# dubhater/vapoursynth-mvtools

Hardware: AMD Instinct MI355X
Metric: MDegrain3 cfg3 fps (Super+Analyse+Degrain end-to-end) (higher is better)
Workload: dtype u16; 1 GPU; 4K YUV420P16 Degrain3 blksize=16 overlap=8 pel=2; batches_in_flight=2

## Files before the change

include/mvtools_amd.h:

```cpp
#ifndef MVTOOLS_AMD_H
#define MVTOOLS_AMD_H

#include <stddef.h>
#include <stdint.h>

#ifdef __cplusplus
extern "C" {
#endif

#define MVX_UNSET (-2147483647 - 1)
#define MVX_ERRLEN 256

#define MVX_OK 0
#define MVX_E_ARG (-1)
#define MVX_E_DEVICE (-2)
#define MVX_E_NOMEM (-3)

const char *mvx_last_error(void);
int mvx_device_count(void);
const char *mvx_version(void);


typedef struct mvx_vector { int32_t x, y; int64_t sad; } mvx_vector;

// ... 570 lines not shown
    float motion[4];
    mvx_depan_stabilise_source prev, next;
} mvx_depan_stabilise_frame_plan;

typedef struct mvx_depan_stabilise mvx_depan_stabilise;

int mvx_depan_stabilise_create(const mvx_depan_stabilise_args *args, const mvx_depan_clip *clip, int num_frames, int data_frames,
                               int64_t fps_num, int64_t fps_den, const ptrdiff_t src_pitch[3], const ptrdiff_t dst_pitch[3],
                               mvx_depan_stabilise **out, char *err);
void mvx_depan_stabilise_destroy(mvx_depan_stabilise *h);
void mvx_depan_stabilise_get_info(const mvx_depan_stabilise *h, mvx_depan_stabilise_info *info);
void mvx_depan_stabilise_get_windows(const mvx_depan_stabilise *h, float *wint, float *winrz, float *winfz);
int mvx_depan_stabilise_window(const mvx_depan_stabilise *h, int n, int *data_first, int *data_last, int *clip_first, int *clip_last);
int mvx_depan_stabilise_plan(const mvx_depan_stabilise *h, int n, const float *motions, mvx_depan_stabilise_frame_plan *plan, char *err);

typedef struct mvx_depan_stabilise_job {
    mvx_depan_stabilise_frame_plan plan;
    const void *cur[3];
    const void *prev[3];
    const void *next[3];
    void *dst[3];
} mvx_depan_stabilise_job;

int mvx_depan_stabilise_frames(mvx_depan_stabilise *h, int nframes, const mvx_depan_stabilise_job *jobs, void *stream);

int mvx_scdetect(const mvx_analysis_data *vectors_data, int64_t thscd1, int32_t thscd2, int n, const void *const *blobs,
                 int32_t *scene_change, void *stream, char *err);

void mvx_scale_thscd(int64_t *thscd1, int32_t *thscd2, const mvx_analysis_data *ad);
int mvx_vectors_size(const mvx_analysis_data *ad);

int mvx_debug_option(const char *name, int value);
void mvx_debug_last_launch(int out[5]);
int mvx_analyse_dct_blocks(mvx_analyse *a, const void *plane, ptrdiff_t pitch, int n, const int32_t *xs, const int32_t *ys, void *out_bytes, void *stream);

void *mvx_dev_alloc(size_t bytes);
void *mvx_dev_alloc_uninit(size_t bytes);
void mvx_dev_free(void *p);
void mvx_dev_pool_limit(size_t bytes);
void mvx_dev_pool_trim(void);
int mvx_dev_mem_info(size_t *free_bytes, size_t *total_bytes);
void *mvx_stream_create(void);
void *mvx_stream_create_priority(int level);
void mvx_stream_destroy(void *stream);
int mvx_copy_to_device(void *dst, ptrdiff_t dst_pitch, const void *src_host, ptrdiff_t src_pitch, size_t row_bytes, size_t rows, void *stream);
int mvx_copy_to_host(void *dst_host, ptrdiff_t dst_pitch, const void *src, ptrdiff_t src_pitch, size_t row_bytes, size_t rows, void *stream);
int mvx_stream_sync(void *stream);
void *mvx_host_alloc_pinned(size_t bytes);
void mvx_host_free_pinned(void *p);
int mvx_upload_2d(void *dst, ptrdiff_t dst_pitch, const void *src_host, ptrdiff_t src_pitch, size_t row_bytes, size_t rows, void *stream);
int mvx_download_2d(void *dst_host, ptrdiff_t dst_pitch, const void *src, ptrdiff_t src_pitch, size_t row_bytes, size_t rows, void *stream);
int mvx_dev_memset(void *dst, int value, size_t bytes, void *stream);
int mvx_set_device(int ordinal);
int mvx_warmup(int staging_buffers);

#ifdef __cplusplus
}
#endif
#endif
```

vapoursynth-mvtools_amd/build.py:

```python
import os
import subprocess
import sys

HERE = os.path.dirname(os.path.abspath(__file__))
CSRC = os.path.join(HERE, "csrc")
OUT = os.path.join(HERE, "libmvtools_amd.so")
SOURCES = ["mvx_api.hip", "mvx_super.hip", "mvx_analyse.hip", "mvx_analyse_any.hip", "mvx_analyse_fdct.hip", "mvx_analyse_u8.hip", "mvx_analyse_u16.hip", "mvx_analyse_spec_u8.hip", "mvx_analyse_spec_u16.hip", "mvx_degrain.hip", "mvx_degrain_n.hip", "mvx_compensate_n.hip", "mvx_flow.hip", "mvx_mask.hip", "mvx_depan.hip", "mvx_depan_fft.hip", "mvx_depan_warp.hip", "mvx_scale_vect.hip"]
FLAGS = ["--offload-arch=gfx950", "-O3", "-std=c++17", "-ffp-contract=off", "-fPIC", "-fvisibility=hidden", "-Wall", "-Wno-inline-asm",
         "-Wno-unused-function", "-Wno-unused-variable"]
if os.environ.get("MVX_DEFS"):
    FLAGS += ["-D" + d for d in os.environ["MVX_DEFS"].split()]
if os.environ.get("MVX_PROFILE"):
    FLAGS.append("-DMVX_PROFILE")


def _hipcc():
    for c in (os.environ.get("HIPCC"), "/opt/rocm/bin/hipcc", "hipcc"):
        if c and (os.path.isabs(c) and os.path.exists(c) or not os.path.isabs(c)):
            return c
    return "hipcc"


VSDIR = os.path.join(HERE, "vsplugin")
VS_PLUGIN = os.path.join(HERE, "libmvtools_vs.so")
VS_HOST = os.path.join(HERE, "mvx_vs_host")


def build_vs(force=False, verbose=False):
    srcs = [os.path.join(VSDIR, f) for f in os.listdir(VSDIR)] + [os.path.join(HERE, "..", "include", "mvtools_amd.h")]
    if not force and all(os.path.exists(o) and all(os.path.getmtime(d) <= os.path.getmtime(o) for d in srcs) for o in (VS_PLUGIN, VS_HOST)):
        return VS_PLUGIN, VS_HOST
    cc = os.environ.get("CC", "gcc")
    cmds = [[cc, "-std=gnu11", "-O2", "-Wall", "-Wextra", "-fPIC", "-shared", "-fvisibility=hidden", os.path.join(VSDIR, "mvtools_vs.c"), "-o", VS_PLUGIN,
             "-L" + HERE, "-lmvtools_amd", "-Wl,-rpath,$ORIGIN", "-lpthread"],
            [cc, "-std=gnu11", "-O2", "-Wall", "-Wextra", os.path.join(VSDIR, "minihost.c"), "-o", VS_HOST, "-ldl"]]
    for cmd in cmds:
        if verbose:
            print(" ".join(cmd))
        subprocess.check_call(cmd)
    return VS_PLUGIN, VS_HOST
# ... 39 lines not shown
```

vapoursynth-mvtools_amd/csrc/mvx_analyse.hip:

```cpp
#include <stdarg.h>
#include <stdlib.h>

#include <algorithm>
#include "mvx_analyse_kernel.h"
#include "mvx_analyse_fast.h"
#include "mvx_analyse_spec.h"
#include "mvx_dct_host.h"
int mvx_analyse_launch_spec_u8(const AParams &P, const ASpecLaunch &S);
int mvx_analyse_launch_spec_u16(const AParams &P, const ASpecLaunch &S);


static thread_local char g_err[512];
void mvx_set_error(const char *fmt, ...) {
    va_list ap;
    va_start(ap, fmt);
    vsnprintf(g_err, sizeof(g_err), fmt, ap);
    va_end(ap);
}
extern "C" __attribute__((visibility("default"))) const char *mvx_last_error(void) { return g_err; }

struct MvxDebug {
    int general = 0;
    int cpw1 = 0;
    int spec = 1;
    int team = -1;
};
static MvxDebug g_dbg;
extern "C" __attribute__((visibility("default"))) int mvx_debug_option(const char *name, int value) {
    struct { const char *n; int *p; } tab[] = { { "general", &g_dbg.general }, { "cpw1", &g_dbg.cpw1 }, { "spec", &g_dbg.spec }, { "team", &g_dbg.team } };
    for (auto &t : tab) if (!strcmp(t.n, name)) { *t.p = value; return MVX_OK; }
    mvx_set_error("mvx_debug_option: unknown option %s", name);
    return MVX_E_ARG;
}

static std::atomic<int> g_lastLaunch[5];
extern "C" __attribute__((visibility("default"))) void mvx_debug_last_launch(int out[5]) {
    for (int i = 0; i < 5; i++) out[i] = g_lastLaunch[i].load();
}

static int A(int v, int d) { return v == MVX_UNSET ? d : v; }

static std::atomic<int> g_dctFloat{0};
extern "C" __attribute__((visibility("default"))) int mvx_enable_dct_float(int on) {
    g_dctFloat.store(on ? 1 : 0);
    return MVX_OK;
}
static bool mvx_is_fdct(const AParams &P) { return P.dctmode >= 1 && P.dctmode <= 4; }
static int mvx_dct_upload(AParams &P, float **dTab) {
    if (!mvx_is_fdct(P) || *dTab) return MVX_OK;
    const std::vector<float> t = mvx_dct_tables(P.blkX, P.blkY);
    HIP_CHECK(hipMalloc((void **)dTab, t.size() * sizeof(float)));
    HIP_CHECK(hipMemcpy(*dTab, t.data(), t.size() * sizeof(float), hipMemcpyHostToDevice));
    P.dctTab = *dTab;
    return MVX_OK;
}

void mvx_divided_data(const mvx_analysis_data *in, mvx_analysis_data *out) {
    *out = *in;
    out->nBlkX = in->nBlkX * 2; out->nBlkY = in->nBlkY * 2;
    out->nBlkSizeX = in->nBlkSizeX / 2; out->nBlkSizeY = in->nBlkSizeY / 2;
    out->nOverlapX = in->nOverlapX / 2; out->nOverlapY = in->nOverlapY / 2;
    out->nLvCount = in->nLvCount + 1;
}

__device__ __forceinline__ int mvx_median3(int a, int b, int c) {
    if (((b <= a) && (a <= c)) || ((c <= a) && (a <= b))) return a;
    if (((a <= b) && (b <= c)) || ((c <= b) && (b <= a))) return b;
    return c;
// ... 230 lines not shown
    (void)hipFree(dXY);
    return rc;
}

extern "C" __attribute__((visibility("default"))) int mvx_analyse_frames(mvx_analyse *a, int njobs, const mvx_analyse_job *jobs, void *stream) {
    if (njobs <= 0) return MVX_OK;
    hipStream_t st = (hipStream_t)stream;
    if (int rc0 = mvx_analyse_device_state(a)) return rc0;
    const AParams &P = a->P;
    mvx_analyse::JobSlot &S = a->slot[a->nextSlot.fetch_add(1) % mvx_analyse::kSlots];
    CallGuard::Scope scope(S.guard, st);
    if ((size_t)njobs > S.cap) {
        if (S.d) (void)hipFree(S.d);
        S.cap = (size_t)njobs * 2;
        HIP_CHECK(hipMalloc((void **)&S.d, S.cap * sizeof(AJob)));
    }
    std::vector<AJob> hj(njobs);
    for (int i = 0; i < njobs; i++) {
        for (int p = 0; p < 3; p++) { hj[i].src[p] = (const unsigned char *)jobs[i].src[p]; hj[i].ref[p] = (const unsigned char *)jobs[i].ref[p]; }
        hj[i].blob = (unsigned char *)jobs[i].blob;
        hj[i].fieldShift = jobs[i].field_shift;
        hj[i].valid = jobs[i].ref[0] != nullptr;
        if (((uintptr_t)jobs[i].blob) & 15) { mvx_set_error("mvx_analyse_frames: blob must be 16-byte aligned"); return MVX_E_ARG; }
    }
    if (!g_dbg.cpw1) std::stable_sort(hj.begin(), hj.end(), [](const AJob &x, const AJob &y) { return (uintptr_t)x.ref[0] > (uintptr_t)y.ref[0]; });
    HIP_CHECK(hipMemcpyAsync(S.d, hj.data(), sizeof(AJob) * njobs, hipMemcpyHostToDevice, st));
    int simds = 0;
    {
        int dev = 0, cus = 0;
        HIP_CHECK(hipGetDevice(&dev));
        HIP_CHECK(hipDeviceGetAttribute(&cus, hipDeviceAttributeMultiprocessorCount, dev));
        simds = 4 * cus;
    }
    auto finish = [&](int fast, int cpw, int syncEvery, int kind) {
        g_lastLaunch[0] = fast; g_lastLaunch[1] = cpw; g_lastLaunch[2] = syncEvery; g_lastLaunch[3] = njobs; g_lastLaunch[4] = kind;
        if (P.divide) hipLaunchKernelGGL(analyse_divide_kernel, dim3((P.lv[0].nBlkX * P.lv[0].nBlkY + 255) / 256, njobs), dim3(256), 0, st, a->dP, S.d);
        HIP_CHECK(hipGetLastError());
        return MVX_OK;
    };
    if (mvx_fast_eligible(P) && !g_dbg.general && !g_dbg.cpw1) {
        int srcB = P.blkX * P.blkY * P.bps + 2 * (P.blkX / 2) * (P.blkY / 2) * P.bps;
        const int fRow = (srcB + 15) & ~15;
        int fMaxBlkX = 0;
        for (int i = 0; i < P.nLevels; i++) if (P.lv[i].nBlkX > fMaxBlkX) fMaxBlkX = P.lv[i].nBlkX;
        const int fBins = 1024;
        int fNeed = fRow + fMaxBlkX * 16;
        if (fNeed < fRow + fBins * 4) fNeed = fRow + fBins * 4;
        const bool stripShape8 = P.bps == 1 && P.blkX == 8 && P.chroma && (P.ovX == 4 || P.ovX == 0) && P.shadow[1] != 0;
        const bool uvOrLumaOnly = P.chroma ? P.shadow[1] != 0 : true;
        const bool stripShape16 = P.bps == 1 && P.blkX == 16 && uvOrLumaOnly && (P.ovX == 8 || P.ovX == 0);
        const bool stripShape = (P.bps == 2 && (P.blkX == 16 || (MVX_STRIP32 && P.blkX == 32)) && uvOrLumaOnly && (P.ovX == P.blkX / 2 || (P.blkX == 16 && P.ovX == 0))) || stripShape8 || stripShape16;
        const int sStrip = (P.bps == 2 && P.blkX == 16) ? 2 * 24 * 128  : (P.bps == 2 && MVX_STRIP32 && P.blkX == 32) ? (P.blkX + P.blkX / 2) * 128 : (P.bps == 1 && P.blkX == 16) ? 24 * 64 : 0;
        const int sSrc = stripShape8 ? 16 + 768 : fRow < sStrip ? sStrip : fRow;
        int sNeed = 0, sTabMax = 0;
        for (int i = 0; i < P.nLevels; i++) {
            const bool smallest = i == P.nLevels - 1;
            const int st = smallest ? (P.nLevels == 1 ? P.searchType : P.searchTypeCoarse) : (i == 0 ? P.searchType : P.searchTypeCoarse);
            const int tabB = (st == SearchHex2 ? SPEC_SLOTS_HEX : SPEC_SLOTS_EXH) * SPEC_STRIDE;
            const int need = sSrc + ((P.lv[i].nBlkX * 8 + 15) & ~15) + tabB;
            if (need > sNeed) sNeed = need;
            if (tabB > sTabMax) sTabMax = tabB;
        }
        if (sNeed < sSrc + fBins * 4) sNeed = sSrc + fBins * 4;
        const int teamShared = (64 + fMaxBlkX * 8 + 255) & ~255;
        const int teamPerWave = ((sSrc + sTabMax < sSrc + fBins * 4 ? sSrc + fBins * 4 : sSrc + sTabMax) + 255) & ~255;
        auto teamThatFits = [&](int team) {
            if (team == 1 || team > 8) team = 0;
// ... 5 lines not shown
        const bool useSpecStrips = useSpec && g_dbg.spec != 3 && stripShape;
        int sTab = 0, sRow = fRow;
        if (useSpec) {
            sRow = sSrc;
            sTab = sSrc + ((fMaxBlkX * 8 + 15) & ~15);
            fNeed = sNeed;
        }
        const int perChain = (fNeed + 255) & ~255;
        auto have = [&](int k) {
            if (P.bps == 2 && P.blkX == 8) return k == 1 || k == 2 || k == 4;
            if (P.bps == 2 && P.blkX == 32) return k >= 1 && k <= 3;
            return k >= 1 && k <= 4;
        };
        int k = njobs > 3 * simds ? 4 : njobs > 2 * simds ? 3 : njobs > simds ? 2 : 1;
        if (useSpecStrips && k > 2) k = 2;
        while (k > 1 && (!have(k) || (long long)perChain * 4 * k > 160 * 1024)) k--;
        if ((long long)perChain * 4 * k <= 160 * 1024) {
            const int cpw = useSpecStrips ? 4 : 4 * k;
            int syncEvery = k >= 2 ? (P.bps == 2 ? 32 : 256) : 0;
            if (useSpecStrips) syncEvery = (stripShape8 || stripShape16) ? 0 : 128;
            const int flags = MVX_FAST_XCD_REMAP | ((P.shadow[1] != 0 && P.chroma) ? MVX_FAST_UV : 0) | (g_dbg.spec == 2 ? MVX_FAST_NOSPEC : 0) | (g_dbg.spec == 3 ? MVX_FAST_NOSTRIP : 0);
            const ALaunch L = { njobs, 0, useSpec ? sRow : fRow, useSpec ? sRow : fRow, fBins, fNeed, simds, cpw, k, syncEvery, k, flags, st, a->dP, S.d };
            int rc;
            const int specSide = ((P.blkX == 16 || stripShape8) && P.ovX == 0) ? 1 : 0;
            const int team = useSpec ? teamThatFits(g_dbg.team >= 0 ? g_dbg.team : mvx_team_default(njobs, simds, useSpecStrips, P.bps)) : 0;
            if (team) {
                ALaunch TL = L;
                TL.ldsRow = teamShared; TL.ldsNeed = teamPerWave; TL.ldsHist = sRow; TL.syncEvery = 0; TL.fast = 2; TL.cpw = 1;
                const ASpecLaunch SL = { TL, sRow, team, specSide };
                rc = P.bps == 1 ? mvx_analyse_launch_spec_u8(P, SL) : mvx_analyse_launch_spec_u16(P, SL);
                if (rc == MVX_OK) return finish(2, team, 0, 3);
                if (rc != 1) return rc;
            }
            if (useSpec) { const ASpecLaunch SL = { L, sTab, 0, specSide }; rc = P.bps == 1 ? mvx_analyse_launch_spec_u8(P, SL) : mvx_analyse_launch_spec_u16(P, SL); }
            else rc = P.bps == 1 ? mvx_analyse_launch_fast_u8(P, L) : mvx_analyse_launch_fast_u16(P, L);
            if (rc == MVX_OK) return finish(k, cpw, syncEvery, useSpec ? 2 : 0);
            if (rc != 1) return rc;
        }
    }
    const bool specialised = P.dctmode == 0 && P.xr == 2 && P.yr == 2 && P.blkX == P.blkY && (P.blkX == 16 || P.blkX == 8 || (P.blkX == 32 && P.bps == 2));
    int cpw = g_dbg.cpw1 ? 1 : 4, wpe = 1;
    if (specialised && !g_dbg.cpw1 && njobs > simds) {
        if (P.bps == 1 && (P.blkX == 8 || P.blkX == 16)) wpe = 2;
        if (P.bps == 1 && P.blkX == 8 && njobs > 2 * simds) wpe = 3;
        if (P.bps == 2 && (P.blkX == 16 || P.blkX == 8 || P.blkX == 32)) { wpe = 2; cpw = 8; }
    }
    int srcBytes = P.blkX * P.blkY * P.bps;
    if (P.chroma) srcBytes += 2 * (P.blkX / P.xr) * (P.blkY / P.yr) * P.bps;
    int ldsRow = (srcBytes + 15) & ~15;
    int maxBlkX = 0;
    for (int i = 0; i < P.nLevels; i++) if (P.lv[i].nBlkX > maxBlkX) maxBlkX = P.lv[i].nBlkX;
    const int histBins = 1024;
    const int ldsHist = ldsRow + maxBlkX * 16;
    int ldsBytes = ldsHist + histBins * 4;
    if (mvx_is_fdct(P)) ldsBytes += mvx_dct_lds_bytes(P.blkX, P.blkY);
    if (ldsBytes > 160 * 1024) { mvx_set_error("mvx_analyse_frames: frame too wide for the LDS row buffer"); return MVX_E_ARG; }
    const int ldsNeed = ldsBytes;
    if (ldsBytes < 33 * 1024) ldsBytes = 33 * 1024;
    while (cpw > 1 && (long long)((ldsNeed + 255) & ~255) * cpw > 160 * 1024) {
        cpw = cpw == 8 ? 4 : 1;
        if (wpe == 3) wpe = 2;
        if (P.bps == 2) wpe = 1;
    }
    const int syncEvery = wpe >= 2 ? 256 : 0;
    const ALaunch L = { njobs, ldsBytes, ldsRow, ldsHist, histBins, ldsNeed, simds, cpw, wpe, syncEvery, 0, 0, st, a->dP, S.d };
    bool off32 = true;
// ... 180 lines not shown
```

vapoursynth-mvtools_amd/csrc/mvx_analyse_spec.h:

```cpp
#pragma once
#include <type_traits>
#include "mvx_analyse_fast.h"

#define SPEC_TB 32
#define SPEC_STRIDE (SPEC_TB * 8 + 8)
#define SPEC_SLOTS_HEX 19
#define SPEC_SLOTS_EXH 29
#define MVX_FAST_NOSTRIP 8
#define MVX_FAST_NOSPEC 4

constexpr int SPEC_SW3 = 12;
#ifdef MVX_SPEC_PROF
#define SPROF_N 20
static __device__ unsigned long long g_specprof[SPROF_N];
#define SPROF(i) do { const long long t1_ = (long long)__builtin_amdgcn_s_memtime(); asm volatile("s_waitcnt lgkmcnt(0)" : : "s"(t1_) : "memory"); sprof[i] += t1_ - sprofT; sprofT = t1_; } while (0)
#else
#define SPROF(i) ((void)0)
#endif
#ifdef MVX_SPEC_PROF
#define SPEC_PROF_DUMP_() do { if (l == 0 && chain == 5 && S.role == 1) for (int i = 0; i < SPROF_N; i++) g_specprof[i] = (unsigned long long)S.sprof[i]; } while (0)
#else
#define SPEC_PROF_DUMP_() ((void)0)
#endif
#ifdef MVX_SPEC_STATS
static __device__ unsigned long long g_specstat[MVX_MAX_LEVELS][8];
#endif

template <int BPS, int BW, bool UV, int SWIN = 12, bool TEAM = false, bool SIDE = false> struct SpecSearcher : FastSearcher<BPS, BW, UV, 48> {
    typedef FastSearcher<BPS, BW, UV, 48> F;
    typedef FGeo<BPS, BW> G;
    using F::P; using F::J; using F::lds; using F::ldsRow; using F::ldsHist; using F::histBins;
    using F::nBlkX; using F::nBlkY; using F::pel; using F::logPel; using F::pw; using F::ph; using F::hpad; using F::vpad;
    using F::srcY; using F::srcU; using F::srcV; using F::refY; using F::refU; using F::refV; using F::srcUV; using F::refUV;
    using F::pitchY; using F::pitchC; using F::pstrideY; using F::pstrideC; using F::shadowY; using F::vectors;
    using F::chroma; using F::searchType; using F::nSearchParam; using F::penaltyNew; using F::penaltyZero; using F::pglobal; using F::badrange; using F::badcount; using F::fieldShift;
    using F::badSAD; using F::LSAD; using F::gmvx; using F::gmvy;
    using F::x0; using F::y0; using F::blkIdx; using F::nDxMin; using F::nDyMin; using F::nDxMax; using F::nDyMax;
    using F::predX; using F::predY; using F::pX; using F::pY; using F::nLambda; using F::bestX; using F::bestY; using F::bestSad;
    int ldsTab;
    int role, nw;
    lds_u8 *shRow;
    LDS_AS int *ctl;
    __device__ __forceinline__ int team_advance(int g, int c0, int lo, int hiE, bool fwd, int stepX, int hps) const {
        auto clampAt = [&](int v, int li) { const int xb = stepX * (c0 + li); return min(max(v, -((xb + hps) << logPel)), ((pw - xb - hpad - BW - hpad + hps) << logPel) - 1); };
        if (clampAt(g, lo) == g && clampAt(g, hiE - 1) == g) return g;
        for (int i = 0; i < hiE - lo; i++) g = clampAt(g, fwd ? lo + i : hiE - 1 - i);
        return g;
    }
    __device__ __forceinline__ void team_wait_ge(int need) const {
#ifdef MVX_TEAM_WATCHDOG
        unsigned spins = 0;
#endif
        while (uni(__hip_atomic_load(ctl, __ATOMIC_ACQUIRE, __HIP_MEMORY_SCOPE_WORKGROUP)) < need) {
            __builtin_amdgcn_s_sleep(2);
#ifdef MVX_TEAM_WATCHDOG
            if (++spins > (1u << 26)) __builtin_trap();
#endif
        }
    }
    __device__ __forceinline__ void team_acquire(int myG, int &px, int &py, int &ps) {
        team_wait_ge(myG);
// ... 178 lines not shown
            a0 = t ? b2 : b0; a1 = t ? b3 : b1; a2 = t ? b0 : b2; a3 = t ? b1 : b3;
        };
        rot(aL0, aL1, aL2, aL3, shA); rot(aC0, aC1, aC2, aC3, shB);
        T.aL[0] = aL0; T.aL[1] = aL1; T.aL[2] = aL2; T.aL[3] = aL3; T.aC[0] = aC0; T.aC[1] = aC1; T.aC[2] = aC2; T.aC[3] = aC3;
    }
    __device__ __forceinline__ static void pat_delta(bool hex, int idx, int &dx, int &dy) {
        dx = 0; dy = 0;
        if (hex) {
            if (idx < 6) { dx = tab8(HEX2X >> 8, idx & 7); dy = tab8(HEX2Y >> 8, idx & 7); }
            else if (idx < 14) { dx = tab8(PACK8(0, 0, -1, 1, -1, -1, 1, 1), idx - 6); dy = tab8(PACK8(-1, 1, 0, 0, -1, 1, -1, 1), idx - 6); }
        } else {
            if (idx < 8) { dx = tab8(PACK8(0, 0, -1, 1, -1, -1, 1, 1), idx); dy = tab8(PACK8(-1, 1, 0, 0, -1, 1, -1, 1), idx); }
            else if (idx < 16) { dx = tab8(PACK8(-1, -1, 0, 0, 1, 1, -2, 2), idx - 8); dy = tab8(PACK8(-2, 2, -2, 2, -2, 2, -1, -1), idx - 8); }
            else if (idx < 24) { dx = tab8(PACK8(-2, 2, -2, 2, -2, -2, 2, 2), idx - 16); dy = tab8(PACK8(0, 0, 1, 1, -2, 2, -2, 2), idx - 16); }
        }
    }

    __device__ __forceinline__ void search_level_spec(int lvl, int globalX, int globalY, GL_AS const GVec *coarse, int coarseBlkX, int coarseBlkY, int coarseLogPel, int syncEvery, bool specEnabled, bool stripEnabled) {
        const int l = lane_id();
        const ALevel &L = P.lv[lvl];
        nBlkX = uni(L.nBlkX); nBlkY = uni(L.nBlkY); pel = uni(L.pel); logPel = uni(L.logPel);
        chroma = uni(P.chroma);
        pw = uni(L.pw); ph = uni(L.ph); hpad = uni(L.hpad); vpad = uni(L.vpad);
        auto uptr = [](const unsigned char *p) { return (gl_u8 *)(unsigned long long)uni((long long)(unsigned long long)p); };
        srcY = uptr(J.src[0] + L.off[0]); refY = uptr(J.ref[0] + L.off[0]);
        srcU = uptr(J.src[1] + L.off[1]); refU = uptr(J.ref[1] + L.off[1]);
        srcV = uptr(J.src[2] + L.off[2]); refV = uptr(J.ref[2] + L.off[2]);
        pitchY = (unsigned)uni((int)P.pitch[0]); pitchC = (unsigned)uni((int)P.pitch[1]); pstrideY = (unsigned)uni((int)L.pstride[0]); pstrideC = (unsigned)uni((int)L.pstride[1]);
        shadowY = (unsigned)uni((int)P.shadow[0]);
        srcUV = uptr(J.src[1] + P.shadow[1] + 2 * L.off[1]); refUV = uptr((J.ref[1] ? J.ref[1] : J.src[1]) + P.shadow[1] + 2 * L.off[1]);
        unsigned char *rec = (unsigned char *)(unsigned long long)uni((long long)(unsigned long long)(J.blob + L.blobOff));
        vectors = (GL_AS GVec *)(rec + 4);
        if (l == 0 && (!TEAM || role == 0)) *(int *)rec = 4 + nBlkX * nBlkY * 16;
        const bool smallestPlane = lvl == P.nLevels - 1;
        if constexpr (TEAM) {
            if (role == 0 && l < 8) ctl[l] = 0;
            this->interpolate(coarse, coarseBlkX, coarseBlkY, coarseLogPel, l + 64 * role, 64 * nw);
        } else this->interpolate(coarse, coarseBlkX, coarseBlkY, coarseLogPel);
        __builtin_amdgcn_fence(__ATOMIC_RELEASE, "workgroup");
        __builtin_amdgcn_fence(__ATOMIC_ACQUIRE, "workgroup");
        __builtin_amdgcn_s_barrier();

        if (smallestPlane) { searchType = P.nLevels == 1 ? P.searchType : P.searchTypeCoarse; nSearchParam = P.nLevels == 1 ? P.nPelSearch : P.nSearchParam; }
        else { searchType = lvl == 0 ? P.searchType : P.searchTypeCoarse; nSearchParam = lvl == 0 ? P.nPelSearch : P.nSearchParam; }
        searchType = uni(searchType); nSearchParam = uni(nSearchParam);
        fieldShift = uni(lvl == 0 ? J.fieldShift : 0);
        badSAD = uni(P.badSAD); badrange = uni(P.badrange); badcount = 0;
        gmvx = pel * globalX; gmvy = pel * globalY + fieldShift;
        int nLambdaLevel = P.lambda / (pel * pel);
        const int nScale = 1 << lvl;
        if (P.plevel == 1) nLambdaLevel = nLambdaLevel * nScale;
        else if (P.plevel == 2) nLambdaLevel = nLambdaLevel * nScale * nScale;
        nLambdaLevel = uni(nLambdaLevel);
        penaltyZero = uni(P.pzero); pglobal = uni(P.global ? P.pglobal : P.pzero); penaltyNew = uni(P.pnew); LSAD = uni((long long)P.lsad);
        const int stepX = uni(P.blkX - P.ovX), stepY = uni(P.blkY - P.ovY);
        const int hps = hpad >> lvl, vps = vpad >> lvl;
        const bool meander = uni(P.meander) != 0;
        LDS_AS v2u *rowbuf = (LDS_AS v2u *)(TEAM ? shRow : lds + ldsRow);
        lds_u8 *tab = TEAM ? lds + ldsTab : lds + ldsRow + ((nBlkX * 8 + 15) & ~15);
        this->pf_setup();
        SPROF(8);
        auto lambda_of = [&](int predSad) {
            const double scale = (double)LSAD / (double)(LSAD + (long long)(predSad >> 1));
            return (int)(long long)((double)(long long)nLambdaLevel * scale * scale);
        };
        const bool hexLevel = searchType == SearchHex2;
        const bool specLevel = specEnabled && !smallestPlane;
        int rdx = 0, rdy = 0;
        if (hexLevel) {
            const int g = l >> 2;
            if (g < 6) { rdx = tab8(HEX2X >> 8, g & 7); rdy = tab8(HEX2Y >> 8, g & 7); }
            else if (g < 14) { rdx = tab8(PACK8(0, 0, -1, 1, -1, -1, 1, 1), g - 6); rdy = tab8(PACK8(-1, 1, 0, 0, -1, 1, -1, 1), g - 6); }
        } else {
            const int g = l >> 1, k = g < 8 ? g : g - 8;
            if (g < 8) { rdx = tab8(PACK8(0, 0, -1, 1, -1, -1, 1, 1), k); rdy = tab8(PACK8(-1, 1, 0, 0, -1, 1, -1, 1), k); }
            else if (g < 16) { rdx = tab8(PACK8(-1, -1, 0, 0, 1, 1, -2, 2), k); rdy = tab8(PACK8(-2, 2, -2, 2, -2, 2, -1, -1), k); }
            else if (g < 24) { rdx = tab8(PACK8(-2, 2, -2, 2, -2, -2, 2, 2), k - 8); rdy = tab8(PACK8(0, 0, 1, 1, -2, 2, -2, 2), k - 8); }
        }
        unsigned sPat = 0, bPat0 = 0, bPat1 = 0;
        {
            constexpr bool side8 = STRIP8_OK && SIDE;
            constexpr bool side16 = SIDE;
            const int gb = side8 ? l >> 3 : STRIP8_OK ? (l >= 45 ? 3 : l >= 30 ? 2 : l >= 15 ? 1 : 0) : side16 ? min(l >> 3, 3) : min(l / LPC, 3);
            for (int q = 0; q < 8; q++) {
                int dx, dy;
                if (q < 4) { pat_delta(hexLevel, STRIP8_OK ? q * 16 + (l >> 2) : q * 8 + (l >> 3), dx, dy); sPat |= (unsigned)((dx & 15) | ((dy & 15) << 4)) << (8 * q); }
                pat_delta(hexLevel, q * (side8 ? 8 : 4) + gb, dx, dy);
                const unsigned b = (unsigned)((dx & 15) | ((dy & 15) << 4)) << (8 * (q & 3));
                if (q < 4) bPat0 |= b; else bPat1 |= b;
            }
        }
#ifdef MVX_SPEC_STATS
        unsigned long long st0 = 0, st1 = 0, st2 = 0, st3 = 0, st4 = 0, st5 = 0, st6 = 0, st7 = 0;
#endif

        int prevX = 0, prevY = 0, prevSad = 0;
        const int syncGroups = syncEvery > 0 ? max(1, (syncEvery + GT / 2) / GT) : 0;
        int syncCount = syncGroups - 1;
        int Gc = 0;
// ... 797 lines not shown
                    if (specRow) gmvx = gEndX;
                    if constexpr (TEAM) {
                        if (act) {
                            typedef unsigned a4v __attribute__((ext_vector_type(4), aligned(4)));
                            const a4v t = {bOut[0], bOut[1], bOut[2], 0u};
                            *(GL_AS a4v *)&vectors[blky * nBlkX + c] = t;
                            rowbuf[c] = v2u{(unsigned)pk((int)bOut[0], (int)bOut[1]), bOut[2]};
                        }
                        team_release(myG + 1, prevX, prevY, prevSad);
                    }
                    SPROF(5);
#ifdef MVX_SPEC_PROF
                    sprof[9] += 1;
#endif
                }
                if (!TEAM && in) {
                    typedef unsigned a4v __attribute__((ext_vector_type(4), aligned(4)));
                    const a4v t = {bOut[0], bOut[1], bOut[2], 0u};
                    *(GL_AS a4v *)&vectors[blky * nBlkX + c] = t;
                    rowbuf[c] = v2u{(unsigned)pk((int)bOut[0], (int)bOut[1]), bOut[2]};
                }
            }
        }
#ifdef MVX_SPEC_STATS
        if (l == 0) { atomicAdd(&g_specstat[lvl][0], st0); atomicAdd(&g_specstat[lvl][1], st1); atomicAdd(&g_specstat[lvl][2], st2); atomicAdd(&g_specstat[lvl][3], st3); atomicAdd(&g_specstat[lvl][4], st4); atomicAdd(&g_specstat[lvl][5], st5); atomicAdd(&g_specstat[lvl][6], st6); atomicAdd(&g_specstat[lvl][7], st7); }
#endif
        SPROF(7);
        __builtin_amdgcn_fence(__ATOMIC_RELEASE, "workgroup");
        __builtin_amdgcn_fence(__ATOMIC_ACQUIRE, "workgroup");
        __builtin_amdgcn_s_barrier();
    }
};

template <int BPS, int BW, int WPE, int MAXCPW, bool UV, bool TEAM = false, bool SIDE = false>
__global__ __launch_bounds__(64 * MAXCPW, WPE) void analyse_spec_kernel(const AParams *Pp, const AJob *jobs, int njobs, int ldsChain, int syncEvery, int ldsRow, int ldsHist, int histBins, int ldsTab, int flags) {
    extern __shared__ __attribute__((aligned(16))) unsigned char smem[];
    const AParams &P = *Pp;
    const int cpw = TEAM ? 1 : (int)(blockDim.x >> 6);
    int wg = (int)blockIdx.x;
    if (flags & MVX_FAST_XCD_REMAP) {
        const int n = (int)gridDim.x, x = wg & 7, slot = wg >> 3;
        wg = x * (n >> 3) + min(x, n & 7) + slot;
    }
    const int wave = uni((int)(threadIdx.x >> 6));
    const int chain = uni(TEAM ? wg : wg * cpw + wave);
    if (chain >= njobs) return;
    const AJob &J = jobs[chain];
    if (!J.blob) return;
    const int l = lane_id();
    int *hdr = (int *)J.blob;
    if (TEAM && wave != 0 && !J.valid) return;
    if (!J.valid) {
        if (l == 0) { hdr[0] = P.blobSize; hdr[1] = 0; }
        for (int lvl = P.nLevels - 1; lvl >= 0; lvl--) {
            const ALevel &L = P.lv[lvl];
            unsigned char *rec = J.blob + L.blobOff;
            const int nBlk = L.nBlkX * L.nBlkY;
            if (l == 0) *(int *)rec = 4 + nBlk * 16;
            GVec *v = (GVec *)(rec + 4);
            for (int i = l; i < nBlk; i += WAVE) { GVec d; d.x = 0; d.y = 0; d.sad = P.verybigSAD; v[i] = d; }
        }
        return;
    }
    if (l == 0 && (!TEAM || wave == 0)) { hdr[0] = P.blobSize; hdr[1] = 1; }
    SpecSearcher<BPS, BW, UV, (WPE <= 2 ? 24 : SPEC_SW3), TEAM, SIDE> S(P, J);
    S.lds = (lds_u8 *)smem + (TEAM ? ldsRow : 0) + wave * ldsChain;
    S.ldsRow = ldsRow; S.ldsHist = ldsHist; S.histBins = histBins; S.ldsTab = ldsTab;
    S.role = wave; S.nw = uni((int)(blockDim.x >> 6)); S.ctl = (LDS_AS int *)((lds_u8 *)smem); S.shRow = (lds_u8 *)smem + 64;
#ifdef MVX_SPEC_PROF
    for (int i = 0; i < SPROF_N; i++) S.sprof[i] = 0;
    S.sprofT = (long long)__builtin_amdgcn_s_memtime();
#endif
    int gx = 0, gy = 0;
    GL_AS const GVec *coarse = nullptr;
    int cbx = 0, cby = 0, clp = 0;
    for (int lvl = P.nLevels - 1; lvl >= 0; lvl--) {
        if (coarse && P.global) S.estimate_global(coarse, cbx * cby, 8192 * P.lv[lvl + 1].pel, &gx, &gy);
        S.search_level_spec(lvl, gx, gy, coarse, cbx, cby, clp, (cpw > 1 && !TEAM) ? syncEvery : 0, !(flags & MVX_FAST_NOSPEC), !(flags & MVX_FAST_NOSTRIP));
        coarse = S.vectors; cbx = P.lv[lvl].nBlkX; cby = P.lv[lvl].nBlkY; clp = P.lv[lvl].logPel;
    }
    SPEC_PROF_DUMP_();
}
#ifdef MVX_SPEC_PROF
#define SPEC_PROF_DUMP() do { if (l == 0 && chain == 5) for (int i = 0; i < SPROF_N; i++) g_specprof[i] = (unsigned long long)S.sprof[i]; } while (0)
#else
#define SPEC_PROF_DUMP() ((void)0)
#endif
#if defined(MVX_SPEC_PROF) && defined(MVX_PROF_EXPORT)
extern "C" __attribute__((visibility("default"))) int mvx_debug_specprof(unsigned long long *out) {
    return hipMemcpyFromSymbol(out, HIP_SYMBOL(g_specprof), sizeof(unsigned long long) * SPROF_N) == hipSuccess ? 0 : -1;
}
#endif
#if defined(MVX_SPEC_STATS) && defined(MVX_PROF_EXPORT)
extern "C" __attribute__((visibility("default"))) int mvx_debug_specstats(unsigned long long *out, int reset) {
    if (hipMemcpyFromSymbol(out, HIP_SYMBOL(g_specstat), sizeof(unsigned long long) * MVX_MAX_LEVELS * 8) != hipSuccess) return -1;
    if (reset) { static unsigned long long z[MVX_MAX_LEVELS * 8]; if (hipMemcpyToSymbol(HIP_SYMBOL(g_specstat), z, sizeof(z)) != hipSuccess) return -1; }
    return 0;
}
#endif

struct ASpecLaunch { ALaunch L; int ldsTab; int team; int side; };
template <int BPS, int BW, int WPE, int MAXCPW, bool UV, bool SIDE = false> static int launch_analyse_spec_uv(const ASpecLaunch &S) {
    const ALaunch &L = S.L;
    const int perChain = (L.ldsNeed + 255) & ~255;
    const int cpw = L.cpw < MAXCPW ? L.cpw : MAXCPW;
    const int lds = perChain * cpw;
    if (lds > 64 * 1024)
        HIP_CHECK(hipFuncSetAttribute((const void *)analyse_spec_kernel<BPS, BW, WPE, MAXCPW, UV, false, SIDE>, hipFuncAttributeMaxDynamicSharedMemorySize, lds));
    hipLaunchKernelGGL((analyse_spec_kernel<BPS, BW, WPE, MAXCPW, UV, false, SIDE>), dim3((L.njobs + cpw - 1) / cpw), dim3(64 * cpw), lds, L.st, L.dP, L.dJobs,
                       L.njobs, perChain, L.syncEvery, L.ldsRow, L.ldsHist, L.histBins, S.ldsTab, L.flags);
    return MVX_OK;
}
template <int BPS, int BW, int WPE, int MAXCPW, bool SIDE = false> static int launch_analyse_spec(const ASpecLaunch &S) {
    if (S.L.flags & MVX_FAST_UV) return launch_analyse_spec_uv<BPS, BW, WPE, MAXCPW, true, SIDE>(S);
    return launch_analyse_spec_uv<BPS, BW, WPE, MAXCPW, false, SIDE>(S);
}
template <int BPS, int BW, int WPE, int MAXCPW, bool UV, bool SIDE = false> static int launch_analyse_spec_team_uv(const ASpecLaunch &S) {
    const ALaunch &L = S.L;
    const int nw = S.team < MAXCPW ? S.team : MAXCPW;
    const int perWave = (L.ldsNeed + 255) & ~255;
    const int lds = L.ldsRow + perWave * nw;
    if (lds > 64 * 1024)
        HIP_CHECK(hipFuncSetAttribute((const void *)analyse_spec_kernel<BPS, BW, WPE, MAXCPW, UV, true, SIDE>, hipFuncAttributeMaxDynamicSharedMemorySize, lds));
    hipLaunchKernelGGL((analyse_spec_kernel<BPS, BW, WPE, MAXCPW, UV, true, SIDE>), dim3(L.njobs), dim3(64 * nw), lds, L.st, L.dP, L.dJobs,
                       L.njobs, perWave, 0, L.ldsRow, L.ldsHist, L.histBins, S.ldsTab, L.flags);
    return MVX_OK;
}
template <int BPS, int BW, int WPE, int MAXCPW, bool SIDE = false> static int launch_analyse_spec_team(const ASpecLaunch &S) {
    if (S.L.flags & MVX_FAST_UV) return launch_analyse_spec_team_uv<BPS, BW, WPE, MAXCPW, true, SIDE>(S);
    return launch_analyse_spec_team_uv<BPS, BW, WPE, MAXCPW, false, SIDE>(S);
}
```

vapoursynth-mvtools_amd/mvtools_amd/__init__.py:

```python
import ctypes as C
import os

import numpy as np

_HERE = os.path.dirname(os.path.abspath(__file__))
_LIBPATH = os.environ.get("MVX_LIB") or os.path.join(os.path.dirname(_HERE), "libmvtools_amd.so")
UNSET = -2147483648
ERRLEN = 256


class MvtoolsError(Exception):
    pass


class AnalysisData(C.Structure):
    _fields_ = [(n, C.c_int32) for n in (
        "nMagicKey", "nVersion", "nBlkSizeX", "nBlkSizeY", "nPel", "nLvCount", "nDeltaFrame", "isBackward", "nCPUFlags",
        "nMotionFlags", "nWidth", "nHeight", "nOverlapX", "nOverlapY", "nBlkX", "nBlkY", "bitsPerSample", "yRatioUV",
        "xRatioUV", "nHPadding", "nVPadding")]


class SuperArgs(C.Structure):
    _fields_ = [(n, C.c_int32) for n in ("width", "height", "bits", "subsampling_w", "subsampling_h", "gray", "hpad", "vpad",
                                         "pel", "levels", "chroma", "sharp", "rfilter")]
# ... 348 lines not shown
        L.mvx_depan_compensate_get_info.restype = None
        L.mvx_depan_compensate_map.argtypes = [C.c_void_p, C.c_int, P(C.c_int), P(C.c_int), P(C.c_int)]
        L.mvx_depan_motion_to_transform.argtypes = [C.c_void_p, C.c_int, P(C.c_float), C.c_int, C.c_int, P(C.c_float), P(C.c_float), C.c_char_p]
        L.mvx_depan_compensate_frames.argtypes = [C.c_void_p, C.c_int, P(DepanCompensateJob), C.c_void_p]
        L.mvx_depan_stabilise_create.argtypes = [P(DepanStabiliseArgs), P(DepanClip), C.c_int, C.c_int, C.c_int64, C.c_int64, P(C.c_ssize_t), P(C.c_ssize_t),
                                                 P(C.c_void_p), C.c_char_p]
        L.mvx_depan_stabilise_destroy.argtypes = [C.c_void_p]
        L.mvx_depan_stabilise_get_info.argtypes = [C.c_void_p, P(DepanStabiliseInfo)]
        L.mvx_depan_stabilise_get_info.restype = None
        L.mvx_depan_stabilise_get_windows.argtypes = [C.c_void_p, P(C.c_float), P(C.c_float), P(C.c_float)]
        L.mvx_depan_stabilise_get_windows.restype = None
        L.mvx_depan_stabilise_window.argtypes = [C.c_void_p, C.c_int, P(C.c_int), P(C.c_int), P(C.c_int), P(C.c_int)]
        L.mvx_depan_stabilise_plan.argtypes = [C.c_void_p, C.c_int, P(C.c_float), P(DepanStabilisePlan), C.c_char_p]
        L.mvx_depan_stabilise_frames.argtypes = [C.c_void_p, C.c_int, P(DepanStabiliseJob), C.c_void_p]
        L.mvx_depan_analyse_create.argtypes = [P(DepanAnalyseArgs), P(AnalysisData), P(DepanClip), P(DepanClip), C.c_int, C.c_int, C.c_int, P(C.c_void_p), C.c_char_p]
        L.mvx_depan_analyse_destroy.argtypes = [C.c_void_p]
        L.mvx_depan_analyse_frames.argtypes = [C.c_void_p, C.c_int, P(C.c_void_p), P(C.c_void_p), C.c_ssize_t, P(C.c_int32), P(DepanMotion), C.c_void_p]
        L.mvx_depan_analyse_host.argtypes = [C.c_void_p, C.c_int, P(C.c_void_p), P(C.c_void_p), C.c_ssize_t, P(C.c_int32), P(DepanMotion)]
        L.mvx_depan_estimate_create.argtypes = [P(DepanEstimateArgs), P(DepanClip), C.c_int, P(C.c_void_p), C.c_char_p]
        L.mvx_depan_estimate_destroy.argtypes = [C.c_void_p]
        L.mvx_depan_estimate_get_info.argtypes = [C.c_void_p, P(DepanEstimateInfo)]
        L.mvx_depan_estimate_get_info.restype = None
        L.mvx_depan_estimate_spectra.argtypes = [C.c_void_p, C.c_int, P(C.c_void_p), C.c_ssize_t, P(C.c_void_p), C.c_void_p]
        L.mvx_depan_estimate_correlate.argtypes = [C.c_void_p, C.c_int, P(C.c_void_p), P(C.c_void_p), P(C.c_int32), P(C.c_int32), P(DepanEstimateResult),
                                                   P(DepanEstimateScan), C.c_void_p]
        L.mvx_depan_estimate_correlate_show.argtypes = [C.c_void_p, C.c_int, P(C.c_void_p), P(C.c_void_p), P(C.c_int32), P(C.c_int32), P(DepanEstimateResult),
                                                        P(DepanEstimateScan), P(C.c_void_p), C.c_ssize_t, C.c_void_p]
        L.mvx_depan_estimate_host_tail.argtypes = [C.c_void_p, C.c_int, P(DepanEstimateScan), P(C.c_int32), P(C.c_int32), P(DepanEstimateResult)]
        L.mvx_depan_estimate_finish.argtypes = [C.c_void_p, C.c_int, P(DepanEstimateResult), P(DepanMotion)]
        L.mvx_scale_thscd.argtypes = [P(C.c_int64), P(C.c_int32), P(AnalysisData)]
        L.mvx_vectors_size.argtypes = [P(AnalysisData)]
        L.mvx_vectors_size.restype = C.c_int
        _lib = L
        for env, opt in (("MVX_GENERAL", "general"), ("MVX_SPEC", "spec"), ("MVX_TEAM", "team")):
            if os.environ.get(env) is not None:
                L.mvx_debug_option(opt.encode(), int(os.environ[env]))
        if os.environ.get("MVX_CPW") == "1":
            L.mvx_debug_option(b"cpw1", 1)
    return _lib


def debug_option(name, value):
    _check(lib().mvx_debug_option(name.encode(), int(value)))


_dct_float = False


def enable_dct_float(on=True):
    global _dct_float
    was = _dct_float
    _check(lib().mvx_enable_dct_float(1 if on else 0))
    _dct_float = bool(on)
    return was


def _u(v):
    return UNSET if v is None else int(v)


def _check(rc, err=None):
    if rc:
        msg = err.value.decode() if err is not None and err.value else lib().mvx_last_error().decode()
        raise MvtoolsError(msg)


def _torch():
# ... 1211 lines not shown
```

Baseline: 976.7 fps.

## Split u16 spec analyse into separate coarse-level and finest-level kernel launches

Measured after the change: 965.7 fps. -1.1%, worse.

```diff
diff --git a/include/mvtools_amd.h b/include/mvtools_amd.h
--- a/include/mvtools_amd.h
+++ b/include/mvtools_amd.h
@@ -626,6 +626,7 @@
 
 int mvx_debug_option(const char *name, int value);
 void mvx_debug_last_launch(int out[5]);
+int mvx_debug_last_launch_count(void);
 int mvx_analyse_dct_blocks(mvx_analyse *a, const void *plane, ptrdiff_t pitch, int n, const int32_t *xs, const int32_t *ys, void *out_bytes, void *stream);
 
 void *mvx_dev_alloc(size_t bytes);
diff --git a/vapoursynth-mvtools_amd/build.py b/vapoursynth-mvtools_amd/build.py
--- a/vapoursynth-mvtools_amd/build.py
+++ b/vapoursynth-mvtools_amd/build.py
@@ -5,7 +5,7 @@
 HERE = os.path.dirname(os.path.abspath(__file__))
 CSRC = os.path.join(HERE, "csrc")
 OUT = os.path.join(HERE, "libmvtools_amd.so")
-SOURCES = ["mvx_api.hip", "mvx_super.hip", "mvx_analyse.hip", "mvx_analyse_any.hip", "mvx_analyse_fdct.hip", "mvx_analyse_u8.hip", "mvx_analyse_u16.hip", "mvx_analyse_spec_u8.hip", "mvx_analyse_spec_u16.hip", "mvx_degrain.hip", "mvx_degrain_n.hip", "mvx_compensate_n.hip", "mvx_flow.hip", "mvx_mask.hip", "mvx_depan.hip", "mvx_depan_fft.hip", "mvx_depan_warp.hip", "mvx_scale_vect.hip"]
+SOURCES = ["mvx_api.hip", "mvx_super.hip", "mvx_analyse.hip", "mvx_analyse_any.hip", "mvx_analyse_fdct.hip", "mvx_analyse_u8.hip", "mvx_analyse_u16.hip", "mvx_analyse_spec_u8.hip", "mvx_analyse_spec_u16.hip", "mvx_analyse_spec_split_u16.hip", "mvx_degrain.hip", "mvx_degrain_n.hip", "mvx_compensate_n.hip", "mvx_flow.hip", "mvx_mask.hip", "mvx_depan.hip", "mvx_depan_fft.hip", "mvx_depan_warp.hip", "mvx_scale_vect.hip"]
 FLAGS = ["--offload-arch=gfx950", "-O3", "-std=c++17", "-ffp-contract=off", "-fPIC", "-fvisibility=hidden", "-Wall", "-Wno-inline-asm",
          "-Wno-unused-function", "-Wno-unused-variable"]
 if os.environ.get("MVX_DEFS"):
diff --git a/vapoursynth-mvtools_amd/csrc/mvx_analyse.hip b/vapoursynth-mvtools_amd/csrc/mvx_analyse.hip
--- a/vapoursynth-mvtools_amd/csrc/mvx_analyse.hip
+++ b/vapoursynth-mvtools_amd/csrc/mvx_analyse.hip
@@ -8,6 +8,7 @@
 #include "mvx_dct_host.h"
 int mvx_analyse_launch_spec_u8(const AParams &P, const ASpecLaunch &S);
 int mvx_analyse_launch_spec_u16(const AParams &P, const ASpecLaunch &S);
+int mvx_analyse_launch_spec_split_u16(const AParams &P, const ASpecLaunch &C, const ASpecLaunch &F);
 
 
 static thread_local char g_err[512];
@@ -24,16 +25,19 @@
     int cpw1 = 0;
     int spec = 1;
     int team = -1;
+    int levelsplit = -1;
 };
 static MvxDebug g_dbg;
 extern "C" __attribute__((visibility("default"))) int mvx_debug_option(const char *name, int value) {
-    struct { const char *n; int *p; } tab[] = { { "general", &g_dbg.general }, { "cpw1", &g_dbg.cpw1 }, { "spec", &g_dbg.spec }, { "team", &g_dbg.team } };
+    struct { const char *n; int *p; } tab[] = { { "general", &g_dbg.general }, { "cpw1", &g_dbg.cpw1 }, { "spec", &g_dbg.spec }, { "team", &g_dbg.team }, { "levelsplit", &g_dbg.levelsplit } };
     for (auto &t : tab) if (!strcmp(t.n, name)) { *t.p = value; return MVX_OK; }
     mvx_set_error("mvx_debug_option: unknown option %s", name);
     return MVX_E_ARG;
 }
 
 static std::atomic<int> g_lastLaunch[5];
+static std::atomic<int> g_lastLaunchCount;
+extern "C" __attribute__((visibility("default"))) int mvx_debug_last_launch_count(void) { return g_lastLaunchCount.load(); }
 extern "C" __attribute__((visibility("default"))) void mvx_debug_last_launch(int out[5]) {
     for (int i = 0; i < 5; i++) out[i] = g_lastLaunch[i].load();
 }
@@ -330,7 +334,8 @@
         HIP_CHECK(hipDeviceGetAttribute(&cus, hipDeviceAttributeMultiprocessorCount, dev));
         simds = 4 * cus;
     }
-    auto finish = [&](int fast, int cpw, int syncEvery, int kind) {
+    auto finish = [&](int fast, int cpw, int syncEvery, int kind, int launches = 1) {
+        g_lastLaunchCount = launches;
         g_lastLaunch[0] = fast; g_lastLaunch[1] = cpw; g_lastLaunch[2] = syncEvery; g_lastLaunch[3] = njobs; g_lastLaunch[4] = kind;
         if (P.divide) hipLaunchKernelGGL(analyse_divide_kernel, dim3((P.lv[0].nBlkX * P.lv[0].nBlkY + 255) / 256, njobs), dim3(256), 0, st, a->dP, S.d);
         HIP_CHECK(hipGetLastError());
@@ -402,6 +407,21 @@
                 if (rc == MVX_OK) return finish(2, team, 0, 3);
                 if (rc != 1) return rc;
             }
+            const bool splitShape = useSpecStrips && (g_dbg.spec == 1 || g_dbg.spec == 5) && P.bps == 2 && P.blkX == 16 && P.blkY == 16 && P.ovX == 8 && P.ovY == 8 && P.chroma && P.shadow[1] != 0 &&
+                                    P.searchType == SearchHex2 && P.searchTypeCoarse == SearchExhaustive && P.nLevels >= 2;
+            if (splitShape && g_dbg.levelsplit != 0 && (g_dbg.levelsplit == 1 || k == 2)) {
+                auto needOf = [&](int from, int to) {
+                    int need = sSrc + fBins * 4;
+                    for (int i = from; i <= to; i++) need = std::max(need, sSrc + ((P.lv[i].nBlkX * 8 + 15) & ~15) + (i == 0 ? SPEC_SLOTS_HEX : SPEC_SLOTS_EXH) * SPEC_STRIDE);
+                    return need;
+                };
+                ALaunch LC = L, LF = L;
+                LC.ldsNeed = needOf(1, P.nLevels - 1); LF.ldsNeed = needOf(0, 0);
+                const ASpecLaunch SC = { LC, sTab, 0, 0 }, SF = { LF, sTab, 0, 0 };
+                rc = mvx_analyse_launch_spec_split_u16(P, SC, SF);
+                if (rc == MVX_OK) return finish(k, cpw, syncEvery, 2, 2);
+                if (rc != 1) return rc;
+            }
             if (useSpec) { const ASpecLaunch SL = { L, sTab, 0, specSide }; rc = P.bps == 1 ? mvx_analyse_launch_spec_u8(P, SL) : mvx_analyse_launch_spec_u16(P, SL); }
             else rc = P.bps == 1 ? mvx_analyse_launch_fast_u8(P, L) : mvx_analyse_launch_fast_u16(P, L);
             if (rc == MVX_OK) return finish(k, cpw, syncEvery, useSpec ? 2 : 0);
diff --git a/vapoursynth-mvtools_amd/csrc/mvx_analyse_spec.h b/vapoursynth-mvtools_amd/csrc/mvx_analyse_spec.h
--- a/vapoursynth-mvtools_amd/csrc/mvx_analyse_spec.h
+++ b/vapoursynth-mvtools_amd/csrc/mvx_analyse_spec.h
@@ -9,6 +9,9 @@
 #define MVX_FAST_NOSTRIP 8
 #define MVX_FAST_NOSPEC 4
 
+#define SPEC_LV_ALL 0
+#define SPEC_LV_COARSE 1
+#define SPEC_LV_FINEST 2
 constexpr int SPEC_SW3 = 12;
 #ifdef MVX_SPEC_PROF
 #define SPROF_N 20
@@ -26,7 +29,7 @@
 static __device__ unsigned long long g_specstat[MVX_MAX_LEVELS][8];
 #endif
 
-template <int BPS, int BW, bool UV, int SWIN = 12, bool TEAM = false, bool SIDE = false> struct SpecSearcher : FastSearcher<BPS, BW, UV, 48> {
+template <int BPS, int BW, bool UV, int SWIN = 12, bool TEAM = false, bool SIDE = false, int LV = 0> struct SpecSearcher : FastSearcher<BPS, BW, UV, 48> {
     typedef FastSearcher<BPS, BW, UV, 48> F;
     typedef FGeo<BPS, BW> G;
     using F::P; using F::J; using F::lds; using F::ldsRow; using F::ldsHist; using F::histBins;
@@ -271,7 +274,7 @@
         unsigned char *rec = (unsigned char *)(unsigned long long)uni((long long)(unsigned long long)(J.blob + L.blobOff));
         vectors = (GL_AS GVec *)(rec + 4);
         if (l == 0 && (!TEAM || role == 0)) *(int *)rec = 4 + nBlkX * nBlkY * 16;
-        const bool smallestPlane = lvl == P.nLevels - 1;
+        const bool smallestPlane = LV != SPEC_LV_FINEST && lvl == P.nLevels - 1;
         if constexpr (TEAM) {
             if (role == 0 && l < 8) ctl[l] = 0;
             this->interpolate(coarse, coarseBlkX, coarseBlkY, coarseLogPel, l + 64 * role, 64 * nw);
@@ -283,6 +286,8 @@
         if (smallestPlane) { searchType = P.nLevels == 1 ? P.searchType : P.searchTypeCoarse; nSearchParam = P.nLevels == 1 ? P.nPelSearch : P.nSearchParam; }
         else { searchType = lvl == 0 ? P.searchType : P.searchTypeCoarse; nSearchParam = lvl == 0 ? P.nPelSearch : P.nSearchParam; }
         searchType = uni(searchType); nSearchParam = uni(nSearchParam);
+        if constexpr (LV == SPEC_LV_FINEST) searchType = SearchHex2;
+        else if constexpr (LV == SPEC_LV_COARSE) searchType = SearchExhaustive;
         fieldShift = uni(lvl == 0 ? J.fieldShift : 0);
         badSAD = uni(P.badSAD); badrange = uni(P.badrange); badcount = 0;
         gmvx = pel * globalX; gmvy = pel * globalY + fieldShift;
@@ -303,7 +308,7 @@
             const double scale = (double)LSAD / (double)(LSAD + (long long)(predSad >> 1));
             return (int)(long long)((double)(long long)nLambdaLevel * scale * scale);
         };
-        const bool hexLevel = searchType == SearchHex2;
+        const bool hexLevel = LV == SPEC_LV_FINEST ? true : LV == SPEC_LV_COARSE ? false : searchType == SearchHex2;
         const bool specLevel = specEnabled && !smallestPlane;
         int rdx = 0, rdy = 0;
         if (hexLevel) {
@@ -1167,7 +1172,7 @@
     }
 };
 
-template <int BPS, int BW, int WPE, int MAXCPW, bool UV, bool TEAM = false, bool SIDE = false>
+template <int BPS, int BW, int WPE, int MAXCPW, bool UV, bool TEAM = false, bool SIDE = false, int LV = SPEC_LV_ALL>
 __global__ __launch_bounds__(64 * MAXCPW, WPE) void analyse_spec_kernel(const AParams *Pp, const AJob *jobs, int njobs, int ldsChain, int syncEvery, int ldsRow, int ldsHist, int histBins, int ldsTab, int flags) {
     extern __shared__ __attribute__((aligned(16))) unsigned char smem[];
     const AParams &P = *Pp;
@@ -1185,6 +1190,7 @@
     const int l = lane_id();
     int *hdr = (int *)J.blob;
     if (TEAM && wave != 0 && !J.valid) return;
+    if (LV == SPEC_LV_FINEST && !J.valid) return;
     if (!J.valid) {
         if (l == 0) { hdr[0] = P.blobSize; hdr[1] = 0; }
         for (int lvl = P.nLevels - 1; lvl >= 0; lvl--) {
@@ -1197,8 +1203,9 @@
         }
         return;
     }
-    if (l == 0 && (!TEAM || wave == 0)) { hdr[0] = P.blobSize; hdr[1] = 1; }
-    SpecSearcher<BPS, BW, UV, (WPE <= 2 ? 24 : SPEC_SW3), TEAM, SIDE> S(P, J);
+    static_assert(LV == SPEC_LV_ALL || !TEAM, "the level split is a form of the one-wave-per-chain launch");
+    if (LV != SPEC_LV_FINEST && l == 0 && (!TEAM || wave == 0)) { hdr[0] = P.blobSize; hdr[1] = 1; }
+    SpecSearcher<BPS, BW, UV, (WPE <= 2 ? 24 : SPEC_SW3), TEAM, SIDE, LV> S(P, J);
     S.lds = (lds_u8 *)smem + (TEAM ? ldsRow : 0) + wave * ldsChain;
     S.ldsRow = ldsRow; S.ldsHist = ldsHist; S.histBins = histBins; S.ldsTab = ldsTab;
     S.role = wave; S.nw = uni((int)(blockDim.x >> 6)); S.ctl = (LDS_AS int *)((lds_u8 *)smem); S.shRow = (lds_u8 *)smem + 64;
@@ -1209,7 +1216,12 @@
     int gx = 0, gy = 0;
     GL_AS const GVec *coarse = nullptr;
     int cbx = 0, cby = 0, clp = 0;
-    for (int lvl = P.nLevels - 1; lvl >= 0; lvl--) {
+    if constexpr (LV == SPEC_LV_FINEST) {
+        coarse = (GL_AS const GVec *)((unsigned char *)(unsigned long long)uni((long long)(unsigned long long)(J.blob + P.lv[1].blobOff)) + 4);
+        cbx = P.lv[1].nBlkX; cby = P.lv[1].nBlkY; clp = P.lv[1].logPel;
+    }
+    const int lvlTop = LV == SPEC_LV_FINEST ? 0 : P.nLevels - 1, lvlBottom = LV == SPEC_LV_COARSE ? 1 : 0;
+    for (int lvl = lvlTop; lvl >= lvlBottom; lvl--) {
         if (coarse && P.global) S.estimate_global(coarse, cbx * cby, 8192 * P.lv[lvl + 1].pel, &gx, &gy);
         S.search_level_spec(lvl, gx, gy, coarse, cbx, cby, clp, (cpw > 1 && !TEAM) ? syncEvery : 0, !(flags & MVX_FAST_NOSPEC), !(flags & MVX_FAST_NOSTRIP));
         coarse = S.vectors; cbx = P.lv[lvl].nBlkX; cby = P.lv[lvl].nBlkY; clp = P.lv[lvl].logPel;
@@ -1235,14 +1247,14 @@
 #endif
 
 struct ASpecLaunch { ALaunch L; int ldsTab; int team; int side; };
-template <int BPS, int BW, int WPE, int MAXCPW, bool UV, bool SIDE = false> static int launch_analyse_spec_uv(const ASpecLaunch &S) {
+template <int BPS, int BW, int WPE, int MAXCPW, bool UV, bool SIDE = false, int LV = SPEC_LV_ALL> static int launch_analyse_spec_uv(const ASpecLaunch &S) {
     const ALaunch &L = S.L;
     const int perChain = (L.ldsNeed + 255) & ~255;
     const int cpw = L.cpw < MAXCPW ? L.cpw : MAXCPW;
     const int lds = perChain * cpw;
     if (lds > 64 * 1024)
-        HIP_CHECK(hipFuncSetAttribute((const void *)analyse_spec_kernel<BPS, BW, WPE, MAXCPW, UV, false, SIDE>, hipFuncAttributeMaxDynamicSharedMemorySize, lds));
-    hipLaunchKernelGGL((analyse_spec_kernel<BPS, BW, WPE, MAXCPW, UV, false, SIDE>), dim3((L.njobs + cpw - 1) / cpw), dim3(64 * cpw), lds, L.st, L.dP, L.dJobs,
+        HIP_CHECK(hipFuncSetAttribute((const void *)analyse_spec_kernel<BPS, BW, WPE, MAXCPW, UV, false, SIDE, LV>, hipFuncAttributeMaxDynamicSharedMemorySize, lds));
+    hipLaunchKernelGGL((analyse_spec_kernel<BPS, BW, WPE, MAXCPW, UV, false, SIDE, LV>), dim3((L.njobs + cpw - 1) / cpw), dim3(64 * cpw), lds, L.st, L.dP, L.dJobs,
                        L.njobs, perChain, L.syncEvery, L.ldsRow, L.ldsHist, L.histBins, S.ldsTab, L.flags);
     return MVX_OK;
 }
diff --git a/vapoursynth-mvtools_amd/csrc/mvx_analyse_spec_split_u16.hip b/vapoursynth-mvtools_amd/csrc/mvx_analyse_spec_split_u16.hip
--- /dev/null
+++ b/vapoursynth-mvtools_amd/csrc/mvx_analyse_spec_split_u16.hip
@@ -0,0 +1,12 @@
+#include "mvx_analyse_kernel.h"
+#include "mvx_analyse_spec.h"
+template <int WPE, int MAXCPW> static int launch_split(const ASpecLaunch &C, const ASpecLaunch &F) {
+    if (int rc = launch_analyse_spec_uv<2, 16, WPE, MAXCPW, true, false, SPEC_LV_COARSE>(C)) return rc;
+    return launch_analyse_spec_uv<2, 16, WPE, MAXCPW, true, false, SPEC_LV_FINEST>(F);
+}
+int mvx_analyse_launch_spec_split_u16(const AParams &P, const ASpecLaunch &C, const ASpecLaunch &F) {
+    if (P.blkX != 16 || C.team || C.side || !(C.L.flags & MVX_FAST_UV)) return 1;
+    if (C.L.fast == 2) return launch_split<2, 8>(C, F);
+    if (C.L.fast == 1) return launch_split<1, 4>(C, F);
+    return 1;
+}
diff --git a/vapoursynth-mvtools_amd/mvtools_amd/__init__.py b/vapoursynth-mvtools_amd/mvtools_amd/__init__.py
--- a/vapoursynth-mvtools_amd/mvtools_amd/__init__.py
+++ b/vapoursynth-mvtools_amd/mvtools_amd/__init__.py
@@ -404,7 +404,7 @@
         L.mvx_vectors_size.argtypes = [P(AnalysisData)]
         L.mvx_vectors_size.restype = C.c_int
         _lib = L
-        for env, opt in (("MVX_GENERAL", "general"), ("MVX_SPEC", "spec"), ("MVX_TEAM", "team")):
+        for env, opt in (("MVX_GENERAL", "general"), ("MVX_SPEC", "spec"), ("MVX_TEAM", "team"), ("MVX_LEVELSPLIT", "levelsplit")):
             if os.environ.get(env) is not None:
                 L.mvx_debug_option(opt.encode(), int(os.environ[env]))
         if os.environ.get("MVX_CPW") == "1":
```
